# zhoupc/CNMF_E

Measured on AMD Instinct MI355X. Metric: cnmfe_iters_per_sec, higher is better.
Workload: dtype f32; 1 GPU; c3: 512x512x10000 fp32 video, K=500, ring_radius=15, 1x1 patches of distribute_data.m (1 resident blocks per GPU), spatial=hals, deconv_flag=false, bg_ssub=1; lanes_per_rank=1, parallelism=patches round-robin over 1 rank(s)

## Files before the change

### cnmf_e_amd/csrc/api.hip

```cpp
#include "common.hpp"
#include <mutex>
#include <hip/hip_fp16.h>
#include <math.h>
#include <dlfcn.h>

namespace cnmfe {
thread_local char g_err[1024] = "";

template <class S> __device__ inline float to_f32(S v) { return (float)v; }
template <> __device__ inline float to_f32<__half>(__half v) { return __half2float(v); }

template <class S>
__global__ void k_convert(const S *__restrict__ src, float *__restrict__ dst, int64_t n) {
    int64_t i = (int64_t)blockIdx.x * blockDim.x + threadIdx.x;
    int64_t stride = (int64_t)gridDim.x * blockDim.x;
    for (; i < n; i += stride) dst[i] = to_f32<S>(src[i]);
}

__global__ void k_ymean(const float *__restrict__ Y, int64_t d_b, int64_t T, double *__restrict__ ym, float *__restrict__ ymf) {
    int64_t q = (int64_t)blockIdx.x * blockDim.x + threadIdx.x;
    if (q >= d_b) return;
    double s0 = 0, s1 = 0, s2 = 0, s3 = 0;
    int64_t t = 0;
    for (; t + 3 < T; t += 4) {
// ... 281 lines not shown
    if (first) *first = first_run_of_row(P, reinterpret_cast<const float *>((const char *)P->stat_host + 64));
    return 0;
}

int ring_first_run(cnmfe_ctx *ctx, Patch *P, bool *first) { return ring_stats_get(ctx, P, nullptr, first); }
int ctx_side_stream(cnmfe_ctx *ctx) {
    if (ctx->side_stream) return 0;
    int prio = 0;
    CK(hipStreamGetPriority(ctx->stream_, &prio));
    hipStream_t s = nullptr;
    CK(hipStreamCreateWithPriority(&s, hipStreamDefault, prio));
    hipLaunchKernelGGL(k_scratch_warm, dim3(1), dim3(64), 0, s, (int *)nullptr, 3);
    hipError_t e = hipStreamSynchronize(s);
    if (e == hipSuccess) e = hipEventCreateWithFlags(&ctx->ev_side_fork, hipEventDisableTiming);
    if (e == hipSuccess) e = hipEventCreateWithFlags(&ctx->ev_side_join, hipEventDisableTiming);
    if (e != hipSuccess) {
        (void)hipStreamDestroy(s);
        if (ctx->ev_side_fork) { (void)hipEventDestroy(ctx->ev_side_fork); ctx->ev_side_fork = nullptr; }
        return fail(CNMFE_EHIP, "side stream of option fit_side: %s", hipGetErrorString(e));
    }
    ctx->side_stream = s;
    return 0;
}
int ctx_errflag(cnmfe_ctx *ctx, int **dflag) {
    if (!ctx->errflag.p) {
        RET(ctx->errflag.ensure(sizeof(int)));
        CK(hipMemsetAsync(ctx->errflag.p, 0, sizeof(int), ctx->st()));
    }
    *dflag = ctx->errflag.as<int>();
    return 0;
}
static int errflag_raise(cnmfe_ctx *ctx, int h, bool taken = false) {
    if (!taken) CK(hipMemsetAsync(ctx->errflag.p, 0, sizeof(int), ctx->st()));
// ... 126 lines not shown
    if (ev_copy_done) (void)hipEventDestroy(ev_copy_done);
    for (auto &g : copy_gens) (void)hipEventDestroy(g.second);
    for (auto e : copy_ev_pool) (void)hipEventDestroy(e);
    cnmfe::pin_register(this, false);
    for (auto *j : tjobs) delete j;
    for (auto e : tickets) (void)hipEventDestroy(e);
    if (ticket_flags) (void)hipHostFree(ticket_flags);
    if (stream_) (void)hipStreamDestroy(stream_);
    for (auto *L : lanes) delete L;
    if (ev_fork) (void)hipEventDestroy(ev_fork);
    if (ev_df) (void)hipEventDestroy(ev_df);
}

void cnmfe_ctx::patches_changed() {
    early.valid = false;
    kept.patch_gone();
    for (cnmfe_lane *L : lanes) L->state.kept.patch_gone();
}
int cnmfe_ctx::activate(int lane) {
    if (lanes.empty() || lane == cur_lane) {
        if (!lanes.empty() && lane != 0 && lanes[lane]->fork_seen != fork_gen) {
            CK(hipStreamWaitEvent(stream_, ev_fork, 0)); lanes[lane]->fork_seen = fork_gen;
        }
        if (!lanes.empty() && lane != 0) lanes[lane]->dirty = true;
        return 0;
    }
    if (lane < 0 || lane >= (int)lanes.size()) return fail(CNMFE_ESTATE, "lane %d of %d", lane, (int)lanes.size());
    if (npseg) flush_copies();
    lanes[cur_lane]->store(*this);
    lanes[lane]->load(*this);
// ... 104 lines not shown
        }
        static bool said = false;
        if (!said) { said = true; fprintf(stderr, "[cnmfe] CNMFE_OPTS applied to every context: %s%s%s\n", applied.empty() ? "(none)" : applied.c_str(), ignored.empty() ? "" : "; not known to this build, ignored: ", ignored.c_str()); }
    }
    return ctx;
}

void cnmfe_destroy(cnmfe_ctx *ctx) {
    if (!ctx) return;
    (void)hipSetDevice(ctx->device);
    (void)ctx->join_lanes();
    (void)hipStreamSynchronize(ctx->st());
    if (ctx->side_stream) { (void)hipStreamSynchronize(ctx->side_stream); (void)hipStreamDestroy(ctx->side_stream); ctx->side_stream = nullptr; }
    if (ctx->ev_side_fork) { (void)hipEventDestroy(ctx->ev_side_fork); ctx->ev_side_fork = nullptr; }
    if (ctx->ev_side_join) { (void)hipEventDestroy(ctx->ev_side_join); ctx->ev_side_join = nullptr; }
    delete ctx;
}

int cnmfe_synchronize(cnmfe_ctx *ctx) {
    if (!ctx) return fail(CNMFE_EINVAL, "null context");
    RET(ctx->join_lanes());
    CK(hipStreamSynchronize(ctx->st()));
    if (ctx->copy_stream) CK(hipStreamSynchronize(ctx->copy_stream));
    return ctx_check_errflag(ctx);
}

int cnmfe_set_option(cnmfe_ctx *ctx, const char *name, int64_t value) {
    if (!ctx || !name) return fail(CNMFE_EINVAL, "null argument");
    static const char *known[] = {"r1_variant", "r1_delta", "r1_lazy", "r1_defer", "r1_virtual", "gram_incremental", "prealloc", "solve_packed", "sweep_dag", "win_i8_planes", "solve_staged", "solve_inv", "solve_inv_terms", "gram_i8", "win_i8", "proj_tiled", "proj_i8", "proj_i8_planes", "ssub_virtual", "temporal_early", "fit_side",
                                  "solve_probe", "r1_probe", "deconv_trace", "trace_long", "host_trace", "debug", nullptr};
    if (!strcmp(name, "lanes")) { RET(lanes_set(ctx, value)); ctx->opts[name] = value; return 0; }
    for (int i = 0; known[i]; ++i) if (!strcmp(known[i], name)) { ctx->opts[name] = value; if (!strcmp(name, "host_trace")) ctx->trace_level = (int)value; return 0; }
    return fail(CNMFE_EINVAL, "unknown option '%s'", name);
}

int cnmfe_get_option(cnmfe_ctx *ctx, const char *name, int64_t *value) {
    if (!ctx || !name || !value) return fail(CNMFE_EINVAL, "null argument");
    const struct { const char *n; int64_t v; } counters[] = {{"temporal_early_hits", ctx->early_hits}, {"temporal_early_drops", ctx->early_drops}, {"temporal_early_declined", ctx->early_declined},
                                                              {"temporal_early_entries", ctx->early.nent}, {"temporal_proj_entries", ctx->last_nent}, {"temporal_nowait", ctx->sweep_nowait},
                                                              {"merge_trace_uploads", ctx->merge_uploads}, {"trace_matrix_uploads", ctx->trace_uploads}, {"init_temporal_levels", ctx->last_nlevels}, {"lanes_live", (int64_t)std::max<size_t>(1, ctx->lanes.size())},
                                                              {"bound_K", ctx->bound_valid ? (int64_t)ctx->bound_K : 0}, {"bound_T", ctx->bound_valid ? ctx->bound_T : 0}};
    for (const auto &c : counters) if (!strcmp(c.n, name)) { *value = c.v; return 0; }
    auto it = ctx->opts.find(name);
    if (it == ctx->opts.end()) return fail(CNMFE_EINVAL, "option '%s' is unknown or was never set (its default holds)", name);
    *value = it->second;
    return 0;
}

int cnmfe_patch_create(cnmfe_ctx *ctx, int patch_id, const int32_t pr[4], const int32_t br[4], int32_t d1, int32_t d2, int64_t T) {
    if (!ctx || !pr || !br) return fail(CNMFE_EINVAL, "null argument");
    if (d1 <= 0 || d2 <= 0 || T <= 0) return fail(CNMFE_EINVAL, "bad dims d1=%d d2=%d T=%lld", d1, d2, (long long)T);
    if (!(1 <= br[0] && br[0] <= pr[0] && pr[0] <= pr[1] && pr[1] <= br[1] && br[1] <= d1 &&
          1 <= br[2] && br[2] <= pr[2] && pr[2] <= pr[3] && pr[3] <= br[3] && br[3] <= d2))
        return fail(CNMFE_EINVAL, "patch [%d %d %d %d] must lie inside block [%d %d %d %d] inside the %dx%d FOV",
                    pr[0], pr[1], pr[2], pr[3], br[0], br[1], br[2], br[3], d1, d2);
    CK(hipSetDevice(ctx->device));
    if (ctx->patches.count(patch_id)) { delete ctx->patches[patch_id]; ctx->patches.erase(patch_id); }
    ctx->patches_changed();
    Patch *P = new Patch();
    P->lane = ctx->lanes.empty() ? 0 : (ctx->patches_created++ % (int)ctx->lanes.size());
    memcpy(P->prect, pr, sizeof(P->prect)); memcpy(P->brect, br, sizeof(P->brect));
    P->d1 = d1; P->d2 = d2; P->T = T;
    P->nr = pr[1] - pr[0] + 1; P->nc = pr[3] - pr[2] + 1;
    P->nr_b = br[1] - br[0] + 1; P->nc_b = br[3] - br[2] + 1;
    P->roff = pr[0] - br[0]; P->coff = pr[2] - br[2];
    P->d = (int64_t)P->nr * P->nc; P->d_b = (int64_t)P->nr_b * P->nc_b;
    int rc = P->Y.ensure((size_t)P->d_b * T * sizeof(float));
    if (rc) { delete P; return rc; }
    if (hipMemsetAsync(P->Y.p, 0, (size_t)P->d_b * T * sizeof(float), ctx->st()) != hipSuccess) { delete P; return fail(CNMFE_EHIP, "hipMemsetAsync of the upload staging failed"); }
    P->frame_seen.assign((size_t)T, 0);
    P->Tc = (T + 3) / 4;
// ... 54 lines not shown
    Patch *P = get_patch(ctx, patch_id);
    if (!P) return fail(CNMFE_ESTATE, "patch %d not created", patch_id);
    CK(hipSetDevice(ctx->device));
    RET(ensure_ymean(ctx, P));
    CK(hipMemcpyAsync(out, P->ymean_d.p, P->d_b * sizeof(double), hipMemcpyDeviceToHost, ctx->st()));
    CK(hipStreamSynchronize(ctx->st()));
    return 0;
}

int cnmfe_ring_init(cnmfe_ctx *ctx, int patch_id, int32_t radius, int32_t num_neighbors) {
    if (!ctx) return fail(CNMFE_EINVAL, "null context");
    Patch *P = get_patch(ctx, patch_id);
    if (!P) return fail(CNMFE_ESTATE, "patch %d not created", patch_id);
    if (radius < 1 || radius > 64) return fail(CNMFE_EINVAL, "ring radius %d out of range", radius);
    CK(hipSetDevice(ctx->device));
    std::vector<int32_t> ndr, ndc;
    ring_offsets(radius, num_neighbors, ndr, ndc);
    const int32_t np_ = (int32_t)ndr.size();
    if (np_ < 1) return fail(CNMFE_EINVAL, "ring of radius %d has no neighbours", radius);
    if (np_ > PMAX_RING) return fail(CNMFE_EUNSUPPORTED, "ring with %d neighbours exceeds the supported %d", np_, PMAX_RING);
    if (radius > 24) return fail(CNMFE_EUNSUPPORTED, "ring radius %d: the block-pair covariance table of the ring regression covers radii <= 24", radius);
    int h = radius;
    if ((P->prect[0] - P->brect[0] < std::min(h, P->prect[0] - 1)) || (P->brect[1] - P->prect[1] < std::min(h, P->d1 - P->prect[1])) ||
        (P->prect[2] - P->brect[2] < std::min(h, P->prect[2] - 1)) || (P->brect[3] - P->prect[3] < std::min(h, P->d2 - P->prect[3])))
        return fail(CNMFE_EINVAL, "block halo is narrower than the ring radius %d", radius);
    P->ring_ready = false;
    P->dr.swap(ndr); P->dc.swap(ndc); P->p = np_; P->radius = radius;
    RET(to_dev(ctx, P->ring_dr, P->dr.data(), P->dr.size()));
    RET(to_dev(ctx, P->ring_dc, P->dc.data(), P->dc.size()));
    RET(P->W.ensure((size_t)P->p * P->d * sizeof(float)));
// ... 44 lines not shown
            if (rr < 1 || rr > P->d1 || cc < 1 || cc > P->d2) continue;
            col[e] = (int32_t)((int64_t)(cc - P->brect[2]) * P->nr_b + (rr - P->brect[0]));
            val[e] = W[(size_t)i * P->d + m];
            ++e;
        }
    }
    rowptr[P->d] = e;
    return 0;
}

int cnmfe_ring_set_values(cnmfe_ctx *ctx, int patch_id, const float *val) {
    if (!ctx || !val) return fail(CNMFE_EINVAL, "null argument");
    Patch *P = get_patch(ctx, patch_id);
    if (!P || !P->ring_ready) return fail(CNMFE_ESTATE, "ring of patch %d not initialised", patch_id);
    CK(hipSetDevice(ctx->device));
    std::vector<float> W((size_t)P->p * P->d, 0.f);
    int64_t e = 0;
    for (int64_t m = 0; m < P->d; ++m) {
        int r = P->prect[0] + (int)(m % P->nr), c = P->prect[2] + (int)(m / P->nr);
        for (int i = 0; i < P->p; ++i) {
            int rr = r + P->dr[i], cc = c + P->dc[i];
            if (rr < 1 || rr > P->d1 || cc < 1 || cc > P->d2) continue;
            W[(size_t)i * P->d + m] = val[e++];
        }
    }
    CK(hipMemcpyAsync(P->W.p, W.data(), W.size() * sizeof(float), hipMemcpyHostToDevice, ctx->st()));
    CK(hipStreamSynchronize(ctx->st()));
    P->stat_valid = false;
    P->residual.invalidate();
    return 0;
// ... 66 lines not shown
    return 0;
}

int cnmfe_fit_ring_model(cnmfe_ctx *ctx, int patch_id, int32_t K, const int64_t *A_colptr, const int32_t *A_rowidx,
                         const float *A_val, const float *C, int c_order, double thresh_outlier, int with_projection,
                         float *b0_out, int64_t info[4]) {
    if (!ctx) return fail(CNMFE_EINVAL, "null context");
    Patch *P = get_patch(ctx, patch_id);
    if (!P || !P->ring_ready) return fail(CNMFE_ESTATE, "ring of patch %d not initialised", patch_id);
    RET(check_csc("A", K, P->d_b, A_colptr, A_rowidx));
    if (K > 0 && ((!A_val && A_colptr[K] > 0) || (!C && c_order != CNMFE_BOUND))) return fail(CNMFE_EINVAL, "null A_val / C");
    CK(hipSetDevice(ctx->device));
    RET(ensure_ymean(ctx, P));
    int64_t dummy[4];
    int rc = bg_fit_ring(ctx, P, K, A_colptr, A_rowidx, A_val, C, c_order, with_projection, b0_out, info ? info : dummy, 0, thresh_outlier);
    P->residual.invalidate();
    return rc;
}

int cnmfe_fit_reserve(cnmfe_ctx *ctx, int patch_id) {
    if (!ctx) return fail(CNMFE_EINVAL, "null context");
    Patch *P = get_patch(ctx, patch_id);
    if (!P || !P->ring_ready) return fail(CNMFE_ESTATE, "ring of patch %d not initialised", patch_id);
    CK(hipSetDevice(ctx->device));
    if (ctx->opt("prealloc", 1) == 0) return 0;
    return bg_reserve(ctx, P);
}

int cnmfe_set_noise(cnmfe_ctx *ctx, int patch_id, const float *sn_block) {
    if (!ctx) return fail(CNMFE_EINVAL, "null context");
    Patch *P = get_patch(ctx, patch_id);
// ... 996 lines not shown
```

### cnmf_e_amd/csrc/bg.hip

```cpp
#include "common.hpp"
#include "ring_solve_core.hpp"
#include "win_proj.hpp"
#include <type_traits>

namespace cnmfe {
static inline bool win_planes3(cnmfe_ctx *ctx, int64_t T16) {
    const int64_t o = ctx->opt("win_i8_planes", 0);
    return o == 3 || (o != 4 && T16 * 16 >= 2048);
}


typedef float float4_t __attribute__((ext_vector_type(4)));

__global__ void __launch_bounds__(256) k_build_bf(const float4 *__restrict__ Y4, int64_t Tc, BgGeom g,
                                                  const int *__restrict__ arow, const int *__restrict__ acol, const float *__restrict__ aval,
                                                  const float *__restrict__ Cc, int64_t ldc, float *__restrict__ bf, int tchunk, double *__restrict__ rs) {
    const int blk = blockIdx.x;
    const int bi = blk % g.nbr, bj = blk / g.nbr;
    const int lp = threadIdx.x;
    const int lr = ((lp >> 4) & 3) * 4 + (lp & 3), lc = (lp >> 6) * 4 + ((lp >> 2) & 3);
    const int rb = bi * BLK + lr, cb = bj * BLK + lc;
    const bool in = rb < g.nr_b && cb < g.nc_b;
    const int64_t q = in ? (int64_t)cb * g.nr_b + rb : 0;
    int e0 = 0, e1 = 0;
// ... 680 lines not shown
    }
    if (f.incr && P->base_valid && P->base_kstride != f.kstride) {
        P->cov_base.swap(P->cov_base_alt); P->rowsum_base.swap(P->rowsum_base_alt);
        std::swap(P->base_valid, P->base_alt_valid); std::swap(P->base_kstride, P->base_alt_kstride);
        P->sys.swap(P->sys_alt); std::swap(P->sys_valid, P->sys_alt_valid);
        P->drop_inverses();
    }
    f.build_base = f.incr && !(P->base_valid && P->base_kstride == f.kstride);
    if (f.build_base) P->drop_systems();
    f.ht.mark("footprint block lists");
    f.use_i8 = (f.build_base || !f.incr) && !f.outl && gram_i8_ok(ctx, f.g.Tp);
    geom_frames(f.g, f.g.Tp, f.use_i8);
    f.keep_pt = f.incr && f.has_a && f.kstride == 1 && !P->derived && !(f.b0_only & 2) && ctx->opt("r1_virtual", 1) != 0;
    if (f.keep_pt) { f.dLp = &P->pt_lp; f.dSlot = &P->pt_slot; P->pt_valid = false; }
}
struct SideScope {
    cnmfe_ctx *ctx; bool inside = false;
    explicit SideScope(cnmfe_ctx *c) : ctx(c) {}
    int fork() {
        int *dErr = nullptr;
        RET(ctx_errflag(ctx, &dErr));
        RET(ctx_side_stream(ctx));
        CK(hipEventRecord(ctx->ev_side_fork, ctx->st()));
        CK(hipStreamWaitEvent(ctx->side_stream, ctx->ev_side_fork, 0));
        return 0;
    }
    int enter() { (void)ctx->st(); std::swap(ctx->stream_, ctx->side_stream); inside = true; return 0; }
    int leave() {
        if (!inside) return 0;
        const hipError_t e = hipEventRecord(ctx->ev_side_join, ctx->st());
        std::swap(ctx->stream_, ctx->side_stream); inside = false;
        CK(e);
        CK(hipStreamWaitEvent(ctx->stream_, ctx->ev_side_join, 0));
        return 0;
    }
    ~SideScope() { if (inside) (void)leave(); }
};
static int fit_side_mode(const RingFit &f) {
    const int64_t m = f.ctx->opt("fit_side", 1);
    return (m == 1 || m == 2) && f.ctx->lanes.empty() && f.incr && f.has_a && !f.build_base ? (int)m : 0;
}
static int fit_side_setup(RingFit &f);

static int fit_queue_projection(RingFit &f, int side = 0) {
    cnmfe_ctx *ctx = f.ctx; Patch *P = f.P; const BgGeom &g = f.g;
    SideScope sc(ctx);
    RET(to_dev(ctx, *f.dLp, f.L.lst_ptr)); RET(to_dev(ctx, f.dLk, f.L.lst_k)); RET(to_dev(ctx, f.dBl, f.L.blall)); RET(f.dCsum.ensure((size_t)f.K * sizeof(double)));
    if (!side) LAUNCH(ctx, "bg_trace_subsum", k_trace_subsum, dim3(f.K), dim3(256), 0, f.dCc.as<float>(), f.ldc, g.Tp, g.kstride, f.dCsum.as<double>());
    const int nb_ = (int)f.L.blall.size(), nbig = (int)f.L.blk_nt[3].size();
    f.nsg = plan::win_segments(nb_);
    f.ut_stride = (int64_t)std::max<size_t>(1, f.L.lst_k.size()) * BLKPX; f.gb_stride = (int64_t)f.nblk * WIN_NLB * WIN_NLB;
    RET(f.dUt.ensure((size_t)f.nsg * f.ut_stride * sizeof(double))); RET(f.dGb.ensure((size_t)f.nsg * f.gb_stride * sizeof(double)));
// ... 311 lines not shown
static int fit_solve(RingFit &f) {
    cnmfe_ctx *ctx = f.ctx;
    const unsigned char *act = f.first_run ? nullptr : f.dActive.as<unsigned char>();
    const int probe = (int)ctx->opt("solve_probe", 0);
    if (f.packed) return fit_solve_packed(f, act, probe);
    RET(fit_win_codes(f));
    CovTab tab = f.covtab(); tab.wcodes = ctx->wcodes.as<int>(); tab.woff = f.reach.woff;
    return solve_launch(ctx, f.P, tab, f.g, ctx->rowsum.as<double>(), act, f.nt, probe, ctx->solve_fill.as<double>());
}

int bg_fit_ring(cnmfe_ctx *ctx, Patch *P, int32_t K, const int64_t *A_colptr, const int32_t *A_rowidx, const float *A_val,
                const float *C, int c_order, int with_projection, float *b0_out, int64_t info[4], int b0_only, double thresh_outlier) {
    RingFit f(ctx, P);
    f.K = K; f.A_colptr = A_colptr; f.A_rowidx = A_rowidx; f.A_val = A_val; f.C = C; f.c_order = c_order; f.b0_only = b0_only; f.thresh_outlier = thresh_outlier; f.T = P->T;
    f.outl = thresh_outlier == thresh_outlier; f.has_a = K > 0 && A_colptr[K] > 0; f.a_empty = K == 0;
    if (f.outl && !P->sn_ready && !(b0_only & 1)) return fail(CNMFE_ESTATE, "fit_ring_model with thresh_outlier needs the noise levels of the block (cnmfe_set_noise)");
    RET(fit_traces_up(f));
    f.ht.mark("traces");
    if (b0_only & 1) {
        RET(fit_upload_csr(f));
        RET(fit_b0(f, bg_geom(P)));
        P->residual.invalidate();
        return 0;
    }
    RET(fit_geometry(f, with_projection));
    fit_lists(f);
    if (f.incr && f.has_a && !f.build_base) RET(fit_queue_projection(f, fit_side_mode(f)));
    f.ht.mark("projection queued");
    if (!f.setup_done) {
        RET(fit_upload_csr(f));
        f.ht.mark("A csr");
        RET(fit_active_b0(f));
        f.ht.mark("ind_active + b0");
    }
    RET(fit_pair_tables(f));
    if (!f.incr || f.build_base) RET(fit_base_table(f));
    if (f.nt < 1 || f.nt > 8) return fail(CNMFE_EUNSUPPORTED, "fit_ring_model: %d ring neighbours (<= %d supported)", P->p, PMAX_RING);
    RET(fit_pack(f));
    if (f.incr) RET(fit_corrections(f, C, c_order));
    f.ht.mark("base / correction launches");
    RET(fit_solve(f));
    RET(ring_stats_enqueue(ctx, P));
    f.ht.mark("solve launch");
    if (b0_out) {
        std::vector<double> tmp(P->d);
        CK(hipMemcpyAsync(tmp.data(), P->b0.p, P->d * sizeof(double), hipMemcpyDeviceToHost, ctx->st()));
        CK(hipStreamSynchronize(ctx->st()));
        for (int64_t i = 0; i < P->d; ++i) b0_out[i] = (float)tmp[i];
        if (f.nactive < 0) f.nactive = *reinterpret_cast<const int *>((const char *)P->stat_host + 8);
    }
    if (info) { info[0] = f.first_run ? 1 : 0; info[1] = f.kstride; info[2] = f.nactive; info[3] = f.pmax; }
    P->residual.invalidate();
    return 0;
}

int win_i8_table(cnmfe_ctx *ctx, Patch *P, const char *name_dig, const char *name_proj, int K, const float *dCc, int64_t ldc, const std::vector<int> &lst_ptr, const std::vector<int> &blall,
                 const int *dLp, const int *dLk, int nsg, double *dUt, int64_t ut_stride) {
    RET(trace_digits(ctx, name_dig, dCc, ldc, K, P->T, P->dig_T16, false));
    return win_proj_i8_launch(ctx, P, name_proj, lst_ptr, blall, dLp, dLk, nsg, dUt, ut_stride);
}

int tu_warm_bg() { hipFuncAttributes at; return hipFuncGetAttributes(&at, (const void *)k_rowsum) == hipSuccess ? 0 : -1; }

}
```

### cnmf_e_amd/csrc/common.hpp

```cpp
#pragma once
#include <hip/hip_runtime.h>
#include <stdint.h>
#include <stdio.h>
#include <stdarg.h>
#include <string.h>
#include <string>
#include <vector>
#include <cstring>
#include <chrono>
#include <cmath>
#include <map>
#include <algorithm>
#include "../../include/cnmfe.h"
#include "ring_plan.hpp"
#include "residual_plan.hpp"
#include "kept_results.hpp"

namespace cnmfe {

typedef unsigned nt_u32x4_t __attribute__((ext_vector_type(4)));
__device__ __forceinline__ uint4 ld_stream(const uint4 *p) {
    const nt_u32x4_t v = __builtin_nontemporal_load(reinterpret_cast<const nt_u32x4_t *>(p));
    return make_uint4(v.x, v.y, v.z, v.w);
}
// ... 111 lines not shown
    bool ac = false; int64_t ldc = 0; int32_t K = 0;
    DevBuf cnt, k, v, cc, cm;
    void set(bool ac_, int64_t ldc_, int32_t K_) { ac = ac_; ldc = ldc_; K = K_; }
    void take(bool ac_, int64_t ldc_, int32_t K_, DevBuf &cnt_, DevBuf &k_, DevBuf &v_, DevBuf &cc_, DevBuf &cm_) {
        set(ac_, ldc_, K_);
        if (ac_) { cnt.swap(cnt_); k.swap(k_); v.swap(v_); cc.swap(cc_); cm.swap(cm_); }
    }
    void swap(FootTerm &o) { std::swap(ac, o.ac); std::swap(ldc, o.ldc); std::swap(K, o.K); cnt.swap(o.cnt); k.swap(o.k); v.swap(o.v); cc.swap(o.cc); cm.swap(o.cm); }
    rplan::TermView view() const { return {ac, ldc, K}; }
};
struct ResidualState {
    rplan::Form form = rplan::NONE;
    int source = rplan::SRC_NONE;
    int64_t gen = 0;
    bool has_pending = false;
    FootTerm applied, pending;
    bool valid() const { return form != rplan::NONE; }
    bool is_virtual() const { return form == rplan::VIRTUAL; }
    void invalidate() { form = rplan::NONE; source = rplan::SRC_NONE; has_pending = false; applied.ac = false; }
    rplan::TermsView terms() const { return {has_pending, applied.view(), pending.view()}; }
};

struct Patch {
    int32_t prect[4], brect[4];
    int32_t d1 = 0, d2 = 0;
    int32_t nr = 0, nc = 0, nr_b = 0, nc_b = 0;
    int32_t roff = 0, coff = 0;
    int64_t T = 0, d = 0, d_b = 0;
    DevBuf Y;
    DevBuf Yc4;
    int64_t Tc = 0;
    DevBuf ymean_d;
    DevBuf ymean_f;
    bool ymean_valid = false;
// ... 133 lines not shown

struct cnmfe_lane {
    cnmfe::LaneState state;
    void store(cnmfe::LaneState &active) { state = std::move(active); }
    void load(cnmfe::LaneState &active) { active = std::move(state); state.stream_ = nullptr; }
    hipEvent_t ev = nullptr; int64_t fork_seen = 0; bool dirty = false;
    ~cnmfe_lane() { if (state.stream_) (void)hipStreamDestroy(state.stream_); if (ev) (void)hipEventDestroy(ev); }
};

struct cnmfe_ctx : cnmfe::LaneState {
    int device = 0;
    void flush_copies();
    hipStream_t st() { if (npseg) flush_copies(); return stream_; }
    hipStream_t copy_stream = nullptr;
    hipStream_t side_stream = nullptr; hipEvent_t ev_side_fork = nullptr, ev_side_join = nullptr;
    hipEvent_t ev_bound_ready = nullptr, ev_copy_done = nullptr; bool copy_pending = false;
    int64_t copy_gen = 0; std::vector<std::pair<int64_t, hipEvent_t>> copy_gens; std::vector<hipEvent_t> copy_ev_pool;
    int copy_batch_mark();
    std::vector<hipEvent_t> tickets; std::vector<char> ticket_busy;
    int *ticket_flags = nullptr;
    cnmfe::DevBuf ticket_dev;
    static constexpr size_t TICKET_FLAGS = 1024;
    cnmfe::Profiler prof;
    std::map<int, cnmfe::Patch *> patches;
    cnmfe::DevBuf bound;
    int32_t bound_K = 0; int64_t bound_T = 0; int bound_order = 1; bool bound_valid = false;
    int64_t bound_gen = 0;
    size_t hw_vp[32] = {}, hw_cc = 0, hw_cm = 0, hw_wa[3] = {0, 0, 0};
    struct LastTemporal { cnmfe::DevBuf craw, aa; int32_t K = 0; int64_t ldc = 0, T = 0; bool valid = false;
        void set(int32_t K_, int64_t ldc_, int64_t T_) { K = K_; ldc = ldc_; T = T_; valid = true; } } last_t;
// ... 159 lines not shown
int peel_open_residual_run(cnmfe_ctx *ctx, Patch *P, int32_t Ksel, const int64_t *A_colptr, const int32_t *A_rowidx, const float *A_val, const float *C, int c_order,
                           const float *psf, int32_t psf_n, float sig, float *Cn_out, float *PNR_out, float *Sn_out, float *Yres_out, int out_memspace);
int peel_open_run(cnmfe_ctx *ctx, Patch *P, const float *psf, int32_t psf_n, int64_t nframes, const double *Q, int32_t M, float sig,
                  float *Cn_out, float *PNR_out, float *Sn_out);
int peel_extract_run(cnmfe_ctx *ctx, Patch *P, int r, int c, int gSiz, double *corr_box, double *ai_box, double *ci_out, double *stats);
int peel_apply_run(cnmfe_ctx *ctx, Patch *P, int r, int c, int gSiz, const double *ai_box, const double *Hai_box2, const double *ci, double sig, double min_pnr,
                   double min_corr, float *PNR_box2, float *Cn_box2);
int spatial_fetch(cnmfe_ctx *ctx, float *A_out, int64_t nnz);
int spatial_fetch_connected(cnmfe_ctx *ctx, int32_t d1, int32_t d2, int32_t K, const int64_t *IND_colptr, const int32_t *IND_rowidx, float *A_out, uint8_t *keep, bool wait = true);
int temporal_early_project(cnmfe_ctx *ctx, int32_t K, const int64_t *IND_colptr, const int32_t *IND_rowidx, int64_t *token);
int ring_first_run(cnmfe_ctx *ctx, Patch *P, bool *first);
int ring_stats_enqueue(cnmfe_ctx *ctx, Patch *P);
int ring_stats_get(cnmfe_ctx *ctx, Patch *P, int *pmax, bool *first);
int center_traces(cnmfe_ctx *ctx, const float *C, int64_t ldc, int32_t K, int64_t T, DevBuf &Cc, DevBuf &Cmean);
int upload_centered(cnmfe_ctx *ctx, DevBuf &stage, const float *C, int32_t K, int64_t T, int order, DevBuf &Cc, DevBuf &Cmean, int64_t *ldc_out);
int ctx_side_stream(cnmfe_ctx *ctx);
int ctx_errflag(cnmfe_ctx *ctx, int **dflag);
int ctx_check_errflag(cnmfe_ctx *ctx);
}
```

### cnmf_e_amd/csrc/kept_results.hpp

```cpp
#pragma once
#include <cstdint>

namespace cnmfe {
struct Patch;
namespace kept {

enum Slot { SCR_COLPTR = 0, SCR_EROW = 1, SCR_AVAL = 6, SCR_KEEP = 14 };

struct KeptSpatial {
    int64_t nnz = -1; const Patch *patch = nullptr; int32_t K = 0; int64_t gen = 0; bool pattern = false, flags = false;
    void record(int64_t nnz_, const Patch *P, int32_t K_, int64_t gen_) { nnz = nnz_; patch = P; K = K_; gen = gen_; pattern = nnz_ > 0; flags = false; }
    void flags_written() { flags = pattern; }
    void drop() { *this = KeptSpatial(); }
    void drop_pattern() { pattern = flags = false; }
    void patch_gone() { patch = nullptr; }
    bool fetchable(int64_t n) const { return nnz >= 0 && n == nnz; }
    bool fetchable_connected(int64_t n) const { return fetchable(n) && (n == 0 || pattern); }
};

struct ProjOpts {
    int64_t i8 = 1, i8_planes = 3, tiled = 1;
    bool operator==(const ProjOpts &o) const { return i8 == o.i8 && i8_planes == o.i8_planes && tiled == o.tiled; }
};

// ... 15 lines not shown
           && E.proj == q.proj;
}
struct ServeRequest {
    int64_t mode; bool one_lane;
    int32_t K; int64_t nnz, spatial_gen;
    bool patch_is_fov, is_virtual, src_full;
};
enum Serve { SERVE_OFF = 0, SERVE_DECLINED = 1, SERVE_YES = 2 };
inline Serve early_serves(const KeptSpatial &k, const ServeRequest &q) {
    if ((q.mode != 1 && q.mode != 2) || !q.one_lane) return SERVE_OFF;
    if (!k.patch || k.K != q.K || q.nnz == 0 || k.nnz != q.nnz || !k.flags || k.gen != q.spatial_gen
        || !q.patch_is_fov || !q.is_virtual || !q.src_full) return SERVE_DECLINED;
    return SERVE_YES;
}

}
}
```

### cnmf_e_amd/csrc/resid.hip

```cpp
#include "common.hpp"

namespace cnmfe {

__global__ void __launch_bounds__(256) k_center_traces(const float *__restrict__ C, int64_t ldc, int64_t T, float *__restrict__ Cc, double *__restrict__ Cmean, const int *__restrict__ idx) {
    int k = blockIdx.x;
    const float4 *row = reinterpret_cast<const float4 *>(C + (int64_t)(idx ? idx[k] : k) * ldc);
    __shared__ double red[4];
    const int64_t n4 = ldc >> 2;
    double s0 = 0, s1 = 0, s2 = 0, s3 = 0;
    for (int64_t c = threadIdx.x; c < n4; c += 256) {
        const float4 v = row[c];
        const int64_t t = 4 * c;
        s0 += v.x; s1 += t + 1 < T ? v.y : 0.f; s2 += t + 2 < T ? v.z : 0.f; s3 += t + 3 < T ? v.w : 0.f;
    }
    double s = (s0 + s1) + (s2 + s3);
    for (int o = 32; o > 0; o >>= 1) s += __shfl_xor(s, o);
    if ((threadIdx.x & 63) == 0) red[threadIdx.x >> 6] = s;
    __syncthreads();
    const double mean = ((red[0] + red[1]) + (red[2] + red[3])) / (double)T;
    if (threadIdx.x == 0) Cmean[k] = mean;
    float4 *out = reinterpret_cast<float4 *>(Cc + (int64_t)k * ldc);
    for (int64_t c = threadIdx.x; c < n4; c += 256) {
        const float4 v = row[c];
        const int64_t t = 4 * c;
// ... 953 lines not shown
    }
    RET(rc);
    if (deferred) *deferred = defer_term;
    return 0;
}

int residual_realize(cnmfe_ctx *ctx, Patch *P) {
    if (!P->residual.is_virtual()) return 0;
    if (P->residual.source == rplan::SRC_SSUB) return ssub_realize(ctx, P);
    RET(P->ysig.ensure((size_t)P->d * P->Tc * sizeof(float4)));
    RET(r1_sweep(ctx, P, P->ysig, false, 4, false, nullptr));
    P->residual.form = rplan::RESIDENT;
    return 0;
}

int residual_run(cnmfe_ctx *ctx, Patch *P, int pid, int32_t Ksel, const int64_t *A_colptr, const int32_t *A_rowidx,
                 const float *A_val, const float *C, int c_order, float *Ysig_out, int out_memspace, DevBuf *outbuf, int tables_only) {
    const int64_t T = P->T;
    ResidualState &rs = P->residual;
    ++rs.gen;
    DevBuf &ysig = outbuf ? *outbuf : P->ysig;
    DevBuf &dC = ctx->tmp[0], &dCc = ctx->tmp[1], &dCm = ctx->tmp[2], &dArow = ctx->tmp[3], &dAcol = ctx->tmp[4], &dAval = ctx->tmp[5],
           &dWaCnt = ctx->tmp[8], &dWaK = ctx->tmp[9], &dWaV = ctx->tmp[10];
    int64_t ldc = 4;
    bool has_ac = Ksel > 0 && A_colptr[Ksel] > 0;
    if (has_ac) {
        RET(upload_centered(ctx, dC, C, Ksel, T, c_order, dCc, dCm, &ldc));
        HostCSR csr; csc_to_csr(P->d_b, Ksel, A_colptr, A_rowidx, A_val, csr);
        RET(to_dev(ctx, dArow, csr.rowptr.data(), csr.rowptr.size()));
        RET(to_dev(ctx, dAcol, csr.col.data(), csr.col.size()));
        RET(to_dev(ctx, dAval, csr.val.data(), csr.val.size()));
        RET(dWaCnt.ensure_hw(P->d * sizeof(int), ctx->hw_wa[0]));
        const int wa_cap = std::max(WA_CAP, std::min((int)Ksel, WA_CAP_MAX));
        RET(dWaK.ensure_hw((size_t)wa_cap * P->d * sizeof(int), ctx->hw_wa[1]));
        RET(dWaV.ensure_hw((size_t)wa_cap * P->d * sizeof(float), ctx->hw_wa[2]));
        int *dErrWa = nullptr;
        RET(ctx_errflag(ctx, &dErrWa));
        const int nnzA = (int)csr.col.size();
        const size_t wa_stage = (size_t)nnzA * 8;
        if (wa_stage <= 96 * 1024) {
            if (wa_stage > 32 * 1024)
                CK(hipFuncSetAttribute((const void *)k_ring_wa<true>, hipFuncAttributeMaxDynamicSharedMemorySize, 96 * 1024));
            LAUNCH(ctx, "r1_ring_wa", k_ring_wa<true>, dim3((unsigned)((P->d + 127) / 128)), dim3(128), wa_stage, P->W.as<float>(), P->d, P->nr, P->nr_b, P->nc_b,
                   P->roff, P->coff, P->p, P->ring_dr.as<int>(), P->ring_dc.as<int>(), dArow.as<int>(), dAcol.as<int>(), dAval.as<float>(), nnzA,
                   dWaCnt.as<int>(), dWaK.as<int>(), dWaV.as<float>(), dErrWa, wa_cap);
        } else
            LAUNCH(ctx, "r1_ring_wa", k_ring_wa<false>, dim3((unsigned)((P->d + 127) / 128)), dim3(128), 0, P->W.as<float>(), P->d, P->nr, P->nr_b, P->nc_b,
                   P->roff, P->coff, P->p, P->ring_dr.as<int>(), P->ring_dc.as<int>(), dArow.as<int>(), dAcol.as<int>(), dAval.as<float>(), nnzA,
                   dWaCnt.as<int>(), dWaK.as<int>(), dWaV.as<float>(), dErrWa, wa_cap);
    }
    const rplan::Plan plan = rplan::residual_plan({rs.form, rs.source, P->ysig.p != nullptr},
                                                  {rplan::SRC_FULL, has_ac, Ysig_out != nullptr, outbuf != nullptr, tables_only != 0, (double)P->d_b * (double)T}, residual_opts(ctx));
    if (plan.tables) { ctx->last_ldc = ldc; return 0; }
    auto pend = [&](int32_t Kt) { rs.has_pending = true; rs.pending.take(has_ac, ldc, Kt, dWaCnt, dWaK, dWaV, dCc, dCm); };
    switch (plan.action) {
    case rplan::PendOnly:
        pend(Ksel);
        return 0;
    case rplan::PendAndFold:
        pend(Ksel);
        RET(residual_materialize(ctx, P));
        if (Ysig_out) RET(ysig_export(ctx, P, ysig, Ysig_out, out_memspace));
        return 0;
    case rplan::Record:
        rs.applied.set(false, ldc, 0); rs.source = rplan::SRC_FULL;
        pend(has_ac ? Ksel : 0); rs.has_pending = has_ac;
        ctx->last_ldc = ldc;
// ... 22 lines not shown
```

Baseline: 101.4 iter/s.

## Precompute ring W·A tables on side stream right after background solve

After the ring-model solve, the ring statistics readback and the W·A table construction (CSR upload through pinned staging plus the k_ring_wa kernel) are now enqueued on a side stream gated by an event. This lets them overlap with later work on the compute stream. The following residual_run checks that A matches the cached copy by memcmp and, if so, reuses the precomputed tables instead of rebuilding them. This adds host-side copying and comparison of A, extra device buffers, and deferred join points at many API entries, which raises the risk of synchronisation mistakes.

```diff
diff --git a/cnmf_e_amd/csrc/api.hip b/cnmf_e_amd/csrc/api.hip
--- a/cnmf_e_amd/csrc/api.hip
+++ b/cnmf_e_amd/csrc/api.hip
@@ -319,9 +319,13 @@
     hipError_t e = hipStreamSynchronize(s);
     if (e == hipSuccess) e = hipEventCreateWithFlags(&ctx->ev_side_fork, hipEventDisableTiming);
     if (e == hipSuccess) e = hipEventCreateWithFlags(&ctx->ev_side_join, hipEventDisableTiming);
+    if (e == hipSuccess) e = hipEventCreateWithFlags(&ctx->ev_ring_solved, hipEventDisableTiming);
+    if (e == hipSuccess) e = hipEventCreateWithFlags(&ctx->ev_ring_join, hipEventDisableTiming);
     if (e != hipSuccess) {
         (void)hipStreamDestroy(s);
         if (ctx->ev_side_fork) { (void)hipEventDestroy(ctx->ev_side_fork); ctx->ev_side_fork = nullptr; }
+        if (ctx->ev_side_join) { (void)hipEventDestroy(ctx->ev_side_join); ctx->ev_side_join = nullptr; }
+        if (ctx->ev_ring_solved) { (void)hipEventDestroy(ctx->ev_ring_solved); ctx->ev_ring_solved = nullptr; }
         return fail(CNMFE_EHIP, "side stream of option fit_side: %s", hipGetErrorString(e));
     }
     ctx->side_stream = s;
@@ -478,6 +482,7 @@
 
 void cnmfe_ctx::patches_changed() {
     early.valid = false;
+    rs_ahead.valid = false;
     kept.patch_gone();
     for (cnmfe_lane *L : lanes) L->state.kept.patch_gone();
 }
@@ -612,12 +617,16 @@
     if (ctx->side_stream) { (void)hipStreamSynchronize(ctx->side_stream); (void)hipStreamDestroy(ctx->side_stream); ctx->side_stream = nullptr; }
     if (ctx->ev_side_fork) { (void)hipEventDestroy(ctx->ev_side_fork); ctx->ev_side_fork = nullptr; }
     if (ctx->ev_side_join) { (void)hipEventDestroy(ctx->ev_side_join); ctx->ev_side_join = nullptr; }
+    if (ctx->ev_ring_solved) { (void)hipEventDestroy(ctx->ev_ring_solved); ctx->ev_ring_solved = nullptr; }
+    if (ctx->ev_ring_join) { (void)hipEventDestroy(ctx->ev_ring_join); ctx->ev_ring_join = nullptr; }
+    if (ctx->rs_pin) { (void)hipHostFree(ctx->rs_pin); ctx->rs_pin = nullptr; ctx->rs_pin_cap = 0; }
     delete ctx;
 }
 
 int cnmfe_synchronize(cnmfe_ctx *ctx) {
     if (!ctx) return fail(CNMFE_EINVAL, "null context");
     RET(ctx->join_lanes());
+    RET(ctx->ring_side_join());
     CK(hipStreamSynchronize(ctx->st()));
     if (ctx->copy_stream) CK(hipStreamSynchronize(ctx->copy_stream));
     return ctx_check_errflag(ctx);
@@ -625,7 +634,7 @@
 
 int cnmfe_set_option(cnmfe_ctx *ctx, const char *name, int64_t value) {
     if (!ctx || !name) return fail(CNMFE_EINVAL, "null argument");
-    static const char *known[] = {"r1_variant", "r1_delta", "r1_lazy", "r1_defer", "r1_virtual", "gram_incremental", "prealloc", "solve_packed", "sweep_dag", "win_i8_planes", "solve_staged", "solve_inv", "solve_inv_terms", "gram_i8", "win_i8", "proj_tiled", "proj_i8", "proj_i8_planes", "ssub_virtual", "temporal_early", "fit_side",
+    static const char *known[] = {"r1_variant", "r1_delta", "r1_lazy", "r1_defer", "r1_virtual", "gram_incremental", "prealloc", "solve_packed", "sweep_dag", "win_i8_planes", "solve_staged", "solve_inv", "solve_inv_terms", "gram_i8", "win_i8", "proj_tiled", "proj_i8", "proj_i8_planes", "ssub_virtual", "temporal_early", "fit_side", "ring_side",
                                   "solve_probe", "r1_probe", "deconv_trace", "trace_long", "host_trace", "debug", nullptr};
     if (!strcmp(name, "lanes")) { RET(lanes_set(ctx, value)); ctx->opts[name] = value; return 0; }
     for (int i = 0; known[i]; ++i) if (!strcmp(known[i], name)) { ctx->opts[name] = value; if (!strcmp(name, "host_trace")) ctx->trace_level = (int)value; return 0; }
@@ -653,6 +662,7 @@
         return fail(CNMFE_EINVAL, "patch [%d %d %d %d] must lie inside block [%d %d %d %d] inside the %dx%d FOV",
                     pr[0], pr[1], pr[2], pr[3], br[0], br[1], br[2], br[3], d1, d2);
     CK(hipSetDevice(ctx->device));
+    if (ctx->ring_side_join() != 0) return CNMFE_EHIP;
     if (ctx->patches.count(patch_id)) { delete ctx->patches[patch_id]; ctx->patches.erase(patch_id); }
     ctx->patches_changed();
     Patch *P = new Patch();
@@ -737,6 +747,7 @@
     if (!P) return fail(CNMFE_ESTATE, "patch %d not created", patch_id);
     if (radius < 1 || radius > 64) return fail(CNMFE_EINVAL, "ring radius %d out of range", radius);
     CK(hipSetDevice(ctx->device));
+    RET(ctx->ring_side_join());
     std::vector<int32_t> ndr, ndc;
     ring_offsets(radius, num_neighbors, ndr, ndc);
     const int32_t np_ = (int32_t)ndr.size();
@@ -811,6 +822,7 @@
     Patch *P = get_patch(ctx, patch_id);
     if (!P || !P->ring_ready) return fail(CNMFE_ESTATE, "ring of patch %d not initialised", patch_id);
     CK(hipSetDevice(ctx->device));
+    RET(ctx->ring_side_join());
     std::vector<float> W((size_t)P->p * P->d, 0.f);
     int64_t e = 0;
     for (int64_t m = 0; m < P->d; ++m) {
@@ -907,7 +919,9 @@
     RET(ensure_ymean(ctx, P));
     int64_t dummy[4];
     int rc = bg_fit_ring(ctx, P, K, A_colptr, A_rowidx, A_val, C, c_order, with_projection, b0_out, info ? info : dummy, 0, thresh_outlier);
+    const bool marked = rc == 0 && P->residual.solve_marked;
     P->residual.invalidate();
+    P->residual.solve_marked = marked;
     return rc;
 }
 
diff --git a/cnmf_e_amd/csrc/bg.hip b/cnmf_e_amd/csrc/bg.hip
--- a/cnmf_e_amd/csrc/bg.hip
+++ b/cnmf_e_amd/csrc/bg.hip
@@ -718,28 +718,6 @@
     f.keep_pt = f.incr && f.has_a && f.kstride == 1 && !P->derived && !(f.b0_only & 2) && ctx->opt("r1_virtual", 1) != 0;
     if (f.keep_pt) { f.dLp = &P->pt_lp; f.dSlot = &P->pt_slot; P->pt_valid = false; }
 }
-struct SideScope {
-    cnmfe_ctx *ctx; bool inside = false;
-    explicit SideScope(cnmfe_ctx *c) : ctx(c) {}
-    int fork() {
-        int *dErr = nullptr;
-        RET(ctx_errflag(ctx, &dErr));
-        RET(ctx_side_stream(ctx));
-        CK(hipEventRecord(ctx->ev_side_fork, ctx->st()));
-        CK(hipStreamWaitEvent(ctx->side_stream, ctx->ev_side_fork, 0));
-        return 0;
-    }
-    int enter() { (void)ctx->st(); std::swap(ctx->stream_, ctx->side_stream); inside = true; return 0; }
-    int leave() {
-        if (!inside) return 0;
-        const hipError_t e = hipEventRecord(ctx->ev_side_join, ctx->st());
-        std::swap(ctx->stream_, ctx->side_stream); inside = false;
-        CK(e);
-        CK(hipStreamWaitEvent(ctx->stream_, ctx->ev_side_join, 0));
-        return 0;
-    }
-    ~SideScope() { if (inside) (void)leave(); }
-};
 static int fit_side_mode(const RingFit &f) {
     const int64_t m = f.ctx->opt("fit_side", 1);
     return (m == 1 || m == 2) && f.ctx->lanes.empty() && f.incr && f.has_a && !f.build_base ? (int)m : 0;
@@ -1081,6 +1059,7 @@
     RingFit f(ctx, P);
     f.K = K; f.A_colptr = A_colptr; f.A_rowidx = A_rowidx; f.A_val = A_val; f.C = C; f.c_order = c_order; f.b0_only = b0_only; f.thresh_outlier = thresh_outlier; f.T = P->T;
     f.outl = thresh_outlier == thresh_outlier; f.has_a = K > 0 && A_colptr[K] > 0; f.a_empty = K == 0;
+    RET(ctx->ring_side_join());
     if (f.outl && !P->sn_ready && !(b0_only & 1)) return fail(CNMFE_ESTATE, "fit_ring_model with thresh_outlier needs the noise levels of the block (cnmfe_set_noise)");
     RET(fit_traces_up(f));
     f.ht.mark("traces");
@@ -1107,7 +1086,19 @@
     if (f.incr) RET(fit_corrections(f, C, c_order));
     f.ht.mark("base / correction launches");
     RET(fit_solve(f));
-    RET(ring_stats_enqueue(ctx, P));
+    bool solve_marked = false;
+    { const int64_t m = ctx->opt("ring_side", 1);
+      if ((m == 1 || m == 2) && !f.outl && ctx->lanes.empty() && ctx->patches.size() == 1) {
+          int *dErrAhead = nullptr;
+          RET(ctx_errflag(ctx, &dErrAhead));
+          RET(ctx_side_stream(ctx));
+          CK(hipEventRecord(ctx->ev_ring_solved, ctx->st()));
+          solve_marked = true;
+          const rplan::ResidualOpts ro = residual_opts(ctx);
+          const bool tables = f.has_a && !P->derived && ro.delta != 0 && ro.lazy != 0;
+          RET(ring_side_ahead(ctx, P, f.K, tables ? &f.csr : nullptr, A_colptr, A_rowidx, A_val, m == 2));
+      } }
+    if (!solve_marked) RET(ring_stats_enqueue(ctx, P));
     f.ht.mark("solve launch");
     if (b0_out) {
         std::vector<double> tmp(P->d);
@@ -1118,6 +1109,7 @@
     }
     if (info) { info[0] = f.first_run ? 1 : 0; info[1] = f.kstride; info[2] = f.nactive; info[3] = f.pmax; }
     P->residual.invalidate();
+    P->residual.solve_marked = solve_marked;
     return 0;
 }
 
diff --git a/cnmf_e_amd/csrc/common.hpp b/cnmf_e_amd/csrc/common.hpp
--- a/cnmf_e_amd/csrc/common.hpp
+++ b/cnmf_e_amd/csrc/common.hpp
@@ -149,10 +149,11 @@
     int source = rplan::SRC_NONE;
     int64_t gen = 0;
     bool has_pending = false;
+    bool solve_marked = false;
     FootTerm applied, pending;
     bool valid() const { return form != rplan::NONE; }
     bool is_virtual() const { return form == rplan::VIRTUAL; }
-    void invalidate() { form = rplan::NONE; source = rplan::SRC_NONE; has_pending = false; applied.ac = false; }
+    void invalidate() { form = rplan::NONE; source = rplan::SRC_NONE; has_pending = false; solve_marked = false; applied.ac = false; }
     rplan::TermsView terms() const { return {has_pending, applied.view(), pending.view()}; }
 };
 
@@ -316,6 +317,23 @@
     hipStream_t st() { if (npseg) flush_copies(); return stream_; }
     hipStream_t copy_stream = nullptr;
     hipStream_t side_stream = nullptr; hipEvent_t ev_side_fork = nullptr, ev_side_join = nullptr;
+    hipEvent_t ev_ring_solved = nullptr, ev_ring_join = nullptr; bool ring_join_pending = false, ring_join_used = false;
+    cnmfe::DevBuf rsd[4]; void *rs_pin = nullptr; size_t rs_pin_cap = 0;
+    struct RingAhead {
+        bool valid = false; const cnmfe::Patch *P = nullptr; int32_t K = 0; std::vector<int64_t> colptr; std::vector<int32_t> rowidx; std::vector<float> val;
+        void keep(const cnmfe::Patch *P_, int32_t K_, const int64_t *cp, const int32_t *ri, const float *va) {
+            P = P_; K = K_; colptr.assign(cp, cp + K_ + 1); rowidx.assign(ri, ri + cp[K_]); val.assign(va, va + cp[K_]); valid = true;
+        }
+        bool is(const cnmfe::Patch *P_, int32_t K_, const int64_t *cp, const int32_t *ri, const float *va) const {
+            return valid && P == P_ && K == K_ && memcmp(colptr.data(), cp, (size_t)(K_ + 1) * sizeof(int64_t)) == 0
+                   && memcmp(rowidx.data(), ri, rowidx.size() * sizeof(int32_t)) == 0 && memcmp(val.data(), va, val.size() * sizeof(float)) == 0;
+        }
+    } rs_ahead;
+    int ring_side_join() {
+        if (!ring_join_pending) return 0;
+        ring_join_pending = false;
+        return hipStreamWaitEvent(st(), ev_ring_join, 0) == hipSuccess ? 0 : cnmfe::fail(CNMFE_EHIP, "ring_side: the compute stream could not wait for the side stream");
+    }
     hipEvent_t ev_bound_ready = nullptr, ev_copy_done = nullptr; bool copy_pending = false;
     int64_t copy_gen = 0; std::vector<std::pair<int64_t, hipEvent_t>> copy_gens; std::vector<hipEvent_t> copy_ev_pool;
     int copy_batch_mark();
@@ -505,7 +523,32 @@
 int ring_stats_get(cnmfe_ctx *ctx, Patch *P, int *pmax, bool *first);
 int center_traces(cnmfe_ctx *ctx, const float *C, int64_t ldc, int32_t K, int64_t T, DevBuf &Cc, DevBuf &Cmean);
 int upload_centered(cnmfe_ctx *ctx, DevBuf &stage, const float *C, int32_t K, int64_t T, int order, DevBuf &Cc, DevBuf &Cmean, int64_t *ldc_out);
+int ring_side_ahead(cnmfe_ctx *ctx, Patch *P, int32_t K, const HostCSR *csr, const int64_t *A_colptr, const int32_t *A_rowidx, const float *A_val, bool join_now);
 int ctx_side_stream(cnmfe_ctx *ctx);
 int ctx_errflag(cnmfe_ctx *ctx, int **dflag);
 int ctx_check_errflag(cnmfe_ctx *ctx);
-}
+struct SideScope {
+    cnmfe_ctx *ctx; bool inside = false, deferred = false;
+    explicit SideScope(cnmfe_ctx *c) : ctx(c) {}
+    int fork() {
+        int *dErr = nullptr;
+        RET(ctx_errflag(ctx, &dErr));
+        RET(ctx_side_stream(ctx));
+        CK(hipEventRecord(ctx->ev_side_fork, ctx->st()));
+        CK(hipStreamWaitEvent(ctx->side_stream, ctx->ev_side_fork, 0));
+        return 0;
+    }
+    int fork_behind(hipEvent_t ev) { deferred = true; CK(hipStreamWaitEvent(ctx->side_stream, ev, 0)); return 0; }
+    int enter() { (void)ctx->st(); std::swap(ctx->stream_, ctx->side_stream); inside = true; return 0; }
+    int leave() {
+        if (!inside) return 0;
+        const hipError_t e = hipEventRecord(deferred ? ctx->ev_ring_join : ctx->ev_side_join, ctx->st());
+        std::swap(ctx->stream_, ctx->side_stream); inside = false;
+        CK(e);
+        if (deferred) { ctx->ring_join_pending = ctx->ring_join_used = true; return 0; }
+        CK(hipStreamWaitEvent(ctx->stream_, ctx->ev_side_join, 0));
+        return 0;
+    }
+    ~SideScope() { if (inside) { (void)leave(); if (deferred) (void)ctx->ring_side_join(); } }
+};
+}
diff --git a/cnmf_e_amd/csrc/kept_results.hpp b/cnmf_e_amd/csrc/kept_results.hpp
--- a/cnmf_e_amd/csrc/kept_results.hpp
+++ b/cnmf_e_amd/csrc/kept_results.hpp
@@ -1,4 +1,5 @@
 #pragma once
+#include <cstddef>
 #include <cstdint>
 
 namespace cnmfe {
@@ -53,5 +54,10 @@
     return SERVE_YES;
 }
 
+struct RingSideRequest { int64_t mode; bool one_lane; size_t npatches; bool solve_marked, has_ac, foreign, tables_only, want_out, recorded; };
+inline bool ring_side_applies(const RingSideRequest &q) {
+    return (q.mode == 1 || q.mode == 2) && q.one_lane && q.npatches == 1 && q.solve_marked && q.has_ac && !q.foreign && !q.tables_only && !q.want_out && q.recorded;
+}
+
 }
 }
diff --git a/cnmf_e_amd/csrc/resid.hip b/cnmf_e_amd/csrc/resid.hip
--- a/cnmf_e_amd/csrc/resid.hip
+++ b/cnmf_e_amd/csrc/resid.hip
@@ -991,43 +991,101 @@
     return 0;
 }
 
+
+static int ring_wa_launch(cnmfe_ctx *ctx, Patch *P, int32_t K, const int *arow, const int *acol, const float *aval, int nnzA, DevBuf &dWaCnt, DevBuf &dWaK, DevBuf &dWaV, int *dErrWa) {
+    const int wa_cap = std::max(WA_CAP, std::min((int)K, WA_CAP_MAX));
+    const size_t wa_stage = (size_t)nnzA * 8;
+    if (wa_stage <= 96 * 1024) {
+        if (wa_stage > 32 * 1024)
+            CK(hipFuncSetAttribute((const void *)k_ring_wa<true>, hipFuncAttributeMaxDynamicSharedMemorySize, 96 * 1024));
+        LAUNCH(ctx, "r1_ring_wa", k_ring_wa<true>, dim3((unsigned)((P->d + 127) / 128)), dim3(128), wa_stage, P->W.as<float>(), P->d, P->nr, P->nr_b, P->nc_b,
+               P->roff, P->coff, P->p, P->ring_dr.as<int>(), P->ring_dc.as<int>(), arow, acol, aval, nnzA,
+               dWaCnt.as<int>(), dWaK.as<int>(), dWaV.as<float>(), dErrWa, wa_cap);
+    } else
+        LAUNCH(ctx, "r1_ring_wa", k_ring_wa<false>, dim3((unsigned)((P->d + 127) / 128)), dim3(128), 0, P->W.as<float>(), P->d, P->nr, P->nr_b, P->nc_b,
+               P->roff, P->coff, P->p, P->ring_dr.as<int>(), P->ring_dc.as<int>(), arow, acol, aval, nnzA,
+               dWaCnt.as<int>(), dWaK.as<int>(), dWaV.as<float>(), dErrWa, wa_cap);
+    return 0;
+}
+static int wa_ensure(cnmfe_ctx *ctx, Patch *P, int32_t K, DevBuf &dWaCnt, DevBuf &dWaK, DevBuf &dWaV) {
+    const int wa_cap = std::max(WA_CAP, std::min((int)K, WA_CAP_MAX));
+    RET(dWaCnt.ensure_hw(P->d * sizeof(int), ctx->hw_wa[0]));
+    RET(dWaK.ensure_hw((size_t)wa_cap * P->d * sizeof(int), ctx->hw_wa[1]));
+    return dWaV.ensure_hw((size_t)wa_cap * P->d * sizeof(float), ctx->hw_wa[2]);
+}
+int ring_side_ahead(cnmfe_ctx *ctx, Patch *P, int32_t K, const HostCSR *csr, const int64_t *A_colptr, const int32_t *A_rowidx, const float *A_val, bool join_now) {
+    cnmfe_ctx::RingAhead &ah = ctx->rs_ahead;
+    ah.valid = false;
+    int *dErrWa = nullptr;
+    RET(ctx_errflag(ctx, &dErrWa));
+    const int *arow = nullptr, *acol = nullptr; const float *aval = nullptr;
+    size_t bytes = 0;
+    if (csr) {
+        const size_t nrp = (csr->rowptr.size() + 3) & ~size_t(3), nz4 = (csr->col.size() + 3) & ~size_t(3);
+        bytes = (nrp + 2 * nz4) * sizeof(int);
+        if (ctx->ring_join_used) CK(hipEventSynchronize(ctx->ev_ring_join));
+        if (ctx->rs_pin_cap < bytes) {
+            if (ctx->rs_pin) { (void)hipHostFree(ctx->rs_pin); ctx->rs_pin = nullptr; ctx->rs_pin_cap = 0; }
+            const size_t want = bytes + bytes / 2;
+            if (hipHostMalloc(&ctx->rs_pin, want, hipHostMallocDefault) != hipSuccess) { ctx->rs_pin = nullptr; return fail(CNMFE_ENOMEM, "ring_side: %zu bytes of pinned staging", want); }
+            ctx->rs_pin_cap = want;
+        }
+        int *h = static_cast<int *>(ctx->rs_pin);
+        memset(h + nrp - 4, 0, 4 * sizeof(int)); memset(h + nrp + nz4 - 4, 0, 4 * sizeof(int)); memset(h + nrp + 2 * nz4 - 4, 0, 4 * sizeof(int));
+        memcpy(h, csr->rowptr.data(), csr->rowptr.size() * sizeof(int));
+        memcpy(h + nrp, csr->col.data(), csr->col.size() * sizeof(int));
+        memcpy(h + nrp + nz4, csr->val.data(), csr->val.size() * sizeof(float));
+        RET(ctx->rsd[0].ensure(bytes));
+        arow = ctx->rsd[0].as<int>(); acol = arow + nrp; aval = reinterpret_cast<const float *>(acol + nz4);
+        RET(wa_ensure(ctx, P, K, ctx->rsd[1], ctx->rsd[2], ctx->rsd[3]));
+    }
+    SideScope sc(ctx);
+    RET(sc.fork_behind(ctx->ev_ring_solved));
+    RET(sc.enter());
+    RET(ring_stats_enqueue(ctx, P));
+    if (csr) {
+        RET(pinned_to_dev(ctx, ctx->rsd[0].p, ctx->rs_pin, bytes));
+        RET(ring_wa_launch(ctx, P, K, arow, acol, aval, (int)csr->col.size(), ctx->rsd[1], ctx->rsd[2], ctx->rsd[3], dErrWa));
+    }
+    RET(sc.leave());
+    if (join_now) RET(ctx->ring_side_join());
+    if (csr) ah.keep(P, K, A_colptr, A_rowidx, A_val);
+    return 0;
+}
+
 int residual_run(cnmfe_ctx *ctx, Patch *P, int pid, int32_t Ksel, const int64_t *A_colptr, const int32_t *A_rowidx,
                  const float *A_val, const float *C, int c_order, float *Ysig_out, int out_memspace, DevBuf *outbuf, int tables_only) {
     const int64_t T = P->T;
     ResidualState &rs = P->residual;
     ++rs.gen;
     DevBuf &ysig = outbuf ? *outbuf : P->ysig;
-    DevBuf &dC = ctx->tmp[0], &dCc = ctx->tmp[1], &dCm = ctx->tmp[2], &dArow = ctx->tmp[3], &dAcol = ctx->tmp[4], &dAval = ctx->tmp[5],
-           &dWaCnt = ctx->tmp[8], &dWaK = ctx->tmp[9], &dWaV = ctx->tmp[10];
+    DevBuf &dC = ctx->tmp[0], &dCc = ctx->tmp[1], &dCm = ctx->tmp[2], &dArow = ctx->tmp[3], &dAcol = ctx->tmp[4], &dAval = ctx->tmp[5];
     int64_t ldc = 4;
     bool has_ac = Ksel > 0 && A_colptr[Ksel] > 0;
+    const rplan::Plan plan = rplan::residual_plan({rs.form, rs.source, P->ysig.p != nullptr},
+                                                  {rplan::SRC_FULL, has_ac, Ysig_out != nullptr, outbuf != nullptr, tables_only != 0, (double)P->d_b * (double)T}, residual_opts(ctx));
+    const bool side = kept::ring_side_applies({ctx->opt("ring_side", 1), ctx->lanes.empty(), ctx->patches.size(), rs.solve_marked, has_ac, outbuf != nullptr, tables_only != 0,
+                                               Ysig_out != nullptr, plan.action == rplan::PendOnly || plan.action == rplan::Record});
+    DevBuf *wa[3] = {&ctx->tmp[8], &ctx->tmp[9], &ctx->tmp[10]};
     if (has_ac) {
         RET(upload_centered(ctx, dC, C, Ksel, T, c_order, dCc, dCm, &ldc));
-        HostCSR csr; csc_to_csr(P->d_b, Ksel, A_colptr, A_rowidx, A_val, csr);
-        RET(to_dev(ctx, dArow, csr.rowptr.data(), csr.rowptr.size()));
-        RET(to_dev(ctx, dAcol, csr.col.data(), csr.col.size()));
-        RET(to_dev(ctx, dAval, csr.val.data(), csr.val.size()));
-        RET(dWaCnt.ensure_hw(P->d * sizeof(int), ctx->hw_wa[0]));
-        const int wa_cap = std::max(WA_CAP, std::min((int)Ksel, WA_CAP_MAX));
-        RET(dWaK.ensure_hw((size_t)wa_cap * P->d * sizeof(int), ctx->hw_wa[1]));
-        RET(dWaV.ensure_hw((size_t)wa_cap * P->d * sizeof(float), ctx->hw_wa[2]));
-        int *dErrWa = nullptr;
-        RET(ctx_errflag(ctx, &dErrWa));
-        const int nnzA = (int)csr.col.size();
-        const size_t wa_stage = (size_t)nnzA * 8;
-        if (wa_stage <= 96 * 1024) {
-            if (wa_stage > 32 * 1024)
-                CK(hipFuncSetAttribute((const void *)k_ring_wa<true>, hipFuncAttributeMaxDynamicSharedMemorySize, 96 * 1024));
-            LAUNCH(ctx, "r1_ring_wa", k_ring_wa<true>, dim3((unsigned)((P->d + 127) / 128)), dim3(128), wa_stage, P->W.as<float>(), P->d, P->nr, P->nr_b, P->nc_b,
-                   P->roff, P->coff, P->p, P->ring_dr.as<int>(), P->ring_dc.as<int>(), dArow.as<int>(), dAcol.as<int>(), dAval.as<float>(), nnzA,
-                   dWaCnt.as<int>(), dWaK.as<int>(), dWaV.as<float>(), dErrWa, wa_cap);
-        } else
-            LAUNCH(ctx, "r1_ring_wa", k_ring_wa<false>, dim3((unsigned)((P->d + 127) / 128)), dim3(128), 0, P->W.as<float>(), P->d, P->nr, P->nr_b, P->nc_b,
-                   P->roff, P->coff, P->p, P->ring_dr.as<int>(), P->ring_dc.as<int>(), dArow.as<int>(), dAcol.as<int>(), dAval.as<float>(), nnzA,
-                   dWaCnt.as<int>(), dWaK.as<int>(), dWaV.as<float>(), dErrWa, wa_cap);
-    }
-    const rplan::Plan plan = rplan::residual_plan({rs.form, rs.source, P->ysig.p != nullptr},
-                                                  {rplan::SRC_FULL, has_ac, Ysig_out != nullptr, outbuf != nullptr, tables_only != 0, (double)P->d_b * (double)T}, residual_opts(ctx));
+        cnmfe_ctx::RingAhead &ah = ctx->rs_ahead;
+        if (side && (int64_t)ah.rowidx.size() == A_colptr[Ksel] && ah.is(P, Ksel, A_colptr, A_rowidx, A_val)) {
+            RET(ctx->ring_side_join());
+            for (int i = 0; i < 3; ++i) wa[i] = &ctx->rsd[1 + i];
+            ah.valid = false;
+        } else {
+            HostCSR csr; csc_to_csr(P->d_b, Ksel, A_colptr, A_rowidx, A_val, csr);
+            RET(to_dev(ctx, dArow, csr.rowptr.data(), csr.rowptr.size()));
+            RET(to_dev(ctx, dAcol, csr.col.data(), csr.col.size()));
+            RET(to_dev(ctx, dAval, csr.val.data(), csr.val.size()));
+            RET(wa_ensure(ctx, P, Ksel, *wa[0], *wa[1], *wa[2]));
+            int *dErrWa = nullptr;
+            RET(ctx_errflag(ctx, &dErrWa));
+            RET(ring_wa_launch(ctx, P, Ksel, dArow.as<int>(), dAcol.as<int>(), dAval.as<float>(), (int)csr.col.size(), *wa[0], *wa[1], *wa[2], dErrWa));
+        }
+    }
+    DevBuf &dWaCnt = *wa[0], &dWaK = *wa[1], &dWaV = *wa[2];
     if (plan.tables) { ctx->last_ldc = ldc; return 0; }
     auto pend = [&](int32_t Kt) { rs.has_pending = true; rs.pending.take(has_ac, ldc, Kt, dWaCnt, dWaK, dWaV, dCc, dCm); };
     switch (plan.action) {
```

New measurement: 104.9 iter/s (median of 6 runs). 1.03x the previous value.
